# haan6/fm-for-online-recommendation

Measured on AMD Instinct MI355X. Metric: samples/sec online-FM (Criteo-39-field, k=16) FTRL-proximal, higher is better.
Workload: dtype f32

## Files before the change

fm-for-online-recommendation_amd/csrc/fmx_kernels.hip:

```cpp

#include <type_traits>

#include "fmx_common.h"

namespace fmxd {

thread_local char g_err[512] = "";

int fail(int code, const char *fmt, ...) {
  va_list ap;
  va_start(ap, fmt);
  vsnprintf(g_err, sizeof(g_err), fmt, ap);
  va_end(ap);
  return code;
}

int check_launch(const char *what) {
  hipError_t e = hipGetLastError();
  if (e != hipSuccess) return fail(FMX_ERR_LAUNCH, "%s: %s", what, hipGetErrorString(e));
  return FMX_OK;
}

}

namespace {

#include "fmx_sort.inc"

__device__ __forceinline__ void st_sc1(float *p, float v) { __hip_atomic_store(p, v, __ATOMIC_RELAXED, __HIP_MEMORY_SCOPE_AGENT); }
__device__ __forceinline__ float ld_sc1(const float *p) {
  return __hip_atomic_load(p, __ATOMIC_RELAXED, __HIP_MEMORY_SCOPE_AGENT);
}
__device__ __forceinline__ float4 ld_sc1_4(const float *p) { return {ld_sc1(p), ld_sc1(p + 1), ld_sc1(p + 2), ld_sc1(p + 3)}; }
typedef float v4f __attribute__((ext_vector_type(4)));
__device__ __forceinline__ void st_sc1_4(float *p, float4 v) {
  const v4f x = {v.x, v.y, v.z, v.w};
  asm volatile("global_store_dwordx4 %0, %1, off sc1\n\ts_nop 1" ::"v"(p), "v"(x) : "memory");
}
__device__ __forceinline__ void store_part_sc1(float *rec, int q, int kp, float4 cV, float4 cA, float cw) {
  st_sc1_4(rec + 4 * q, cV);
  st_sc1_4(rec + kp + 4 * q, cA);
  if (q == 0) st_sc1(rec + 2 * kp, cw);
}

struct FwdArgs {
  const float *rows;
  const int64_t *foff;
  const float *bias;
  const int32_t *idx;
  const float *xv;
  const float *y;
  fmx_fwd_out_t out;
  fmx_hyper_t h;
  int32_t B, F, kp, stride, zoff, loss_kind;
  int32_t ldS, ld1;
  float inv_b;
  const int32_t *fcols, *fbase;
  int32_t Fc;
};

template <int LPR, int LAYOUT>
__device__ __forceinline__ void forward_finish(const FwdArgs &a, const int b, const int lane, float4 s, float4 ss, float fo, bool bad,
                                               const float y_early, const float bias0_early, const float bias1_early) {
  const int q = lane % LPR;
  const int kp = LPR * 4;
  if (bad && a.out.error) *a.out.error = 1;

#define FMX_BFLY(M)                               \
  if (LPR <= M) {                                 \
    s = s + xor_lane_f4<M>(s, lane);              \
    ss = ss + xor_lane_f4<M>(ss, lane);           \
    fo += xor_lane_f<M>(fo, lane);                \
  }
  FMX_BFLY(1) FMX_BFLY(2) FMX_BFLY(4) FMX_BFLY(8) FMX_BFLY(16) FMX_BFLY(32)
#undef FMX_BFLY
  const float4 bi = 0.5f * (s * s - ss);
  float sbi = (bi.x + bi.y) + (bi.z + bi.w);
#pragma unroll
  for (int m = 1; m < LPR; m <<= 1) sbi += __shfl_xor(sbi, m);
  fo = __shfl(fo, 0);

  if (lane < LPR) {
    if (a.out.S) *reinterpret_cast<float4 *>(a.out.S + (size_t)b * a.ldS + 4 * q) = s;
    if (a.out.bi) *reinterpret_cast<float4 *>(a.out.bi + (size_t)b * kp + 4 * q) = bi;
  }
  if (lane == 0) {
    float bias;
    if (LAYOUT == FMX_LAYOUT_WEIGHTS) bias = bias0_early;
    else bias = ftrl_w(bias0_early, bias1_early, a.h);
    const float z = fo + sbi + bias;
    if (a.out.sfirst) a.out.sfirst[b] = fo;
    if (a.out.sbi) a.out.sbi[b] = sbi;
    if (a.out.logit) a.out.logit[b] = z;
    if (a.loss_kind != FMX_LOSS_NONE) {
      const float y = y_early;
      float loss, dz;
      if (a.loss_kind == FMX_LOSS_BCE_LOGITS) {
        loss = bcewl(z, y);
        dz = (sigmoidf_(z) - y) * a.inv_b;
      } else {
        const float p = sigmoidf_(z);
        loss = bcewl(p, y);
        dz = (sigmoidf_(p) - y) * p * (1.f - p) * a.inv_b;
      }
      if (a.out.loss) a.out.loss[(size_t)b * a.ld1] = loss;
      if (a.out.dz) a.out.dz[(size_t)b * a.ld1] = dz;
    }
  }
}

template <int LPR, int LAYOUT, int NPASS, bool MAPPED = false>
__device__ __forceinline__ void forward_sample(const FwdArgs &a, const int b, const int lane) {
  constexpr int SLOTS = WAVE / LPR;
  constexpr int NP = NPASS > 0 ? NPASS : 1;
  const int slot = lane / LPR, q = lane % LPR;
  const int kp = LPR * 4;

  float4 s = splat(0.f), ss = splat(0.f);
  float fo = 0.f;
  bool bad = false;
  const float y_early = a.loss_kind != FMX_LOSS_NONE ? a.y[b] : 0.f;
  const float bias0_early = a.bias[0];
  const float bias1_early = LAYOUT == FMX_LAYOUT_WEIGHTS ? 0.f : a.bias[1];
  __builtin_amdgcn_sched_barrier(0);
  const int n_outer = NPASS > 0 ? 1 : (a.F + SLOTS - 1) / SLOTS;
  for (int it = 0; it < n_outer; ++it) {
    uint32_t li[NP];
    float x[NP];
    int64_t lo[NP];
    uint32_t vocab[NP];
    bool live[NP];
    const float *xsrc = a.xv ? a.xv : reinterpret_cast<const float *>(a.idx);
    const bool has_x = a.xv != nullptr;
    float xl[NP];
    int64_t hi[NP];
    int fc[NP];
#pragma unroll
    for (int p = 0; p < NP; ++p) {
      const int f = (it * NP + p) * SLOTS + slot;
      live[p] = f < a.F;
      fc[p] = live[p] ? f : a.F - 1;
    }
#pragma unroll
    for (int p = 0; p < NP; ++p) {
      lo[p] = a.foff[fc[p]];
      hi[p] = a.foff[fc[p] + 1];
    }
#pragma unroll
    for (int p = 0; p < NP; ++p) {
      size_t o = (size_t)b * a.F + fc[p];
      uint32_t fb = 0u;
      if (MAPPED) {
        o = (size_t)b * a.Fc + (a.fcols ? a.fcols[fc[p]] : fc[p]);
        fb = a.fbase ? (uint32_t)a.fbase[fc[p]] : 0u;
      }
      li[p] = (uint32_t)a.idx[o] - fb;
      xl[p] = xsrc[o];
    }
#pragma unroll
    for (int p = 0; p < NP; ++p) {
      x[p] = has_x ? xl[p] : 1.f;
      vocab[p] = (uint32_t)(hi[p] - lo[p]);
    }
    float4 r0[NP];
    float rw[NP];
    bool ok[NP];
#pragma unroll
    for (int p = 0; p < NP; ++p) {
      ok[p] = live[p] && li[p] < vocab[p];
      const float *rp = a.rows + (size_t)(lo[p] + (ok[p] ? li[p] : 0u)) * a.stride;
      r0[p] = *reinterpret_cast<const float4 *>(rp + 4 * q);
      rw[p] = rp[kp];
    }
    __builtin_amdgcn_sched_barrier(0);
#pragma unroll
    for (int p = 0; p < NP; ++p) {
      const float4 e = x[p] * r0[p];
      const float f1 = ok[p] ? rw[p] * x[p] : 0.f;
      if (ok[p]) {
        s = s + e;
        ss = ss + e * e;
        fo += f1;
      }
      bad = bad || (!MAPPED && live[p] && !ok[p]);
      if (live[p] && a.out.first && q == 0) a.out.first[(size_t)b * a.F + (it * NP + p) * SLOTS + slot] = f1;
    }
  }
  forward_finish<LPR, LAYOUT>(a, b, lane, s, ss, fo, bad, y_early, bias0_early, bias1_early);
}

template <int LPR, int LAYOUT, int NPASS, bool MAPPED = false>
__global__ __launch_bounds__(256) void k_fm_forward(FwdArgs a) {
  __builtin_amdgcn_s_setprio(3);
  const int b = blockIdx.x * (blockDim.x >> 6) + (threadIdx.x >> 6);
  if (b >= a.B) return;
  forward_sample<LPR, LAYOUT, NPASS, MAPPED>(a, b, threadIdx.x & 63);
}

struct PartArgs {
  const float *rows;
  const int64_t *foff;
  const int32_t *fcols, *fbase;
  const int32_t *idx;
  const float *xv;
  float *rec;
  int32_t *error;
  int32_t B, F, Fc, stride, sl_log2, group;
};

template <int LPR, int NPASS>
__global__ __launch_bounds__(256) void k_fm_forward_part(PartArgs a) {
  constexpr int SLOTS = WAVE / LPR;
  constexpr int kp = LPR * 4, REC = 2 * kp + 4;
  const int lane = threadIdx.x & 63;
  const int slot = lane / LPR, q = lane % LPR;
  const int SL = 1 << a.sl_log2;
  const int slot_l = slot & (SL - 1);
  const int wave = blockIdx.x * (blockDim.x >> 6) + (threadIdx.x >> 6);
  const int b = wave * (SLOTS >> a.sl_log2) + (slot >> a.sl_log2);
  const bool valid = b < a.B;
  const int f0 = (int)blockIdx.y * NPASS * SL;
  const bool pieces = a.fcols || a.fbase;
  uint32_t li[NPASS], vocab[NPASS];
  float x[NPASS], xl[NPASS];
  int64_t lo[NPASS], hi[NPASS];
  bool live[NPASS], ok[NPASS];
  int fc[NPASS];
  const float *xsrc = a.xv ? a.xv : reinterpret_cast<const float *>(a.idx);
  const bool has_x = a.xv != nullptr;
  const int bc = valid ? b : 0;
#pragma unroll
  for (int p = 0; p < NPASS; ++p) {
    const int f = f0 + p * SL + slot_l;
    live[p] = valid && f < a.F;
    fc[p] = f < a.F ? f : a.F - 1;
  }
  int colp[NPASS];
  uint32_t fb[NPASS];
#pragma unroll
  for (int p = 0; p < NPASS; ++p) {
    lo[p] = a.foff[fc[p]];
    hi[p] = a.foff[fc[p] + 1];
    colp[p] = a.fcols ? a.fcols[fc[p]] : fc[p];
    fb[p] = a.fbase ? (uint32_t)a.fbase[fc[p]] : 0u;
  }
#pragma unroll
  for (int p = 0; p < NPASS; ++p) {
    const size_t o = (size_t)bc * a.Fc + colp[p];
    li[p] = (uint32_t)a.idx[o] - fb[p];
    xl[p] = xsrc[o];
  }
#pragma unroll
  for (int p = 0; p < NPASS; ++p) {
    x[p] = has_x ? xl[p] : 1.f;
    vocab[p] = (uint32_t)(hi[p] - lo[p]);
  }
  float4 r0[NPASS];
  float rw[NPASS];
#pragma unroll
  for (int p = 0; p < NPASS; ++p) {
    ok[p] = live[p] && li[p] < vocab[p];
    const float *rp = a.rows + (size_t)(lo[p] + (ok[p] ? li[p] : 0u)) * a.stride;
    r0[p] = *reinterpret_cast<const float4 *>(rp + 4 * q);
    rw[p] = rp[kp];
  }
  __builtin_amdgcn_sched_barrier(0);
  float4 s = splat(0.f), ss = splat(0.f);
  float fo = 0.f;
  bool bad = false;
#pragma unroll
  for (int p = 0; p < NPASS; ++p) {
    const float4 e = x[p] * r0[p];
    if (ok[p]) {
      s = s + e;
      ss = ss + e * e;
      fo += rw[p] * x[p];
    }
    bad = bad || (!pieces && live[p] && !ok[p]);
  }
  if (bad && a.error) *a.error = 1;
#define FMX_BFLY_L(M)                              \
  if (LPR <= M && (M / LPR) < SL) {                \
    s = s + xor_lane_f4<M>(s, lane);               \
    ss = ss + xor_lane_f4<M>(ss, lane);            \
    fo += xor_lane_f<M>(fo, lane);                 \
  }
  FMX_BFLY_L(1) FMX_BFLY_L(2) FMX_BFLY_L(4) FMX_BFLY_L(8) FMX_BFLY_L(16) FMX_BFLY_L(32)
#undef FMX_BFLY_L
  if (valid && slot_l == 0) {
    const int dst = b / a.group;
    float *r = a.rec + (((size_t)dst * gridDim.y + blockIdx.y) * a.group + (b - dst * a.group)) * REC;
    *reinterpret_cast<float4 *>(r + 4 * q) = s;
    *reinterpret_cast<float4 *>(r + kp + 4 * q) = ss;
    if (q == 0) *reinterpret_cast<float4 *>(r + 2 * kp) = float4{fo, 0.f, 0.f, 0.f};
  }
}

struct FinishArgs {
  const float *parts;
  int64_t rank_stride;
  const float *bias;
  const float *y;
  fmx_fwd_out_t out;
  fmx_hyper_t h;
  int32_t B, loss_kind, ldS, ld1;
  float inv_b;
};

template <int LPR, int LAYOUT, int G>
__global__ __launch_bounds__(256) void k_fm_forward_finish(FinishArgs a) {
  constexpr int SLOTS = WAVE / LPR;
  constexpr int kp = LPR * 4, REC = 2 * kp + 4;
  const int lane = threadIdx.x & 63;
  const int slot = lane / LPR, q = lane % LPR;
  const int b = (blockIdx.x * (blockDim.x >> 6) + (threadIdx.x >> 6)) * SLOTS + slot;
  const bool valid = b < a.B;
  const float y_early = (valid && a.loss_kind != FMX_LOSS_NONE) ? a.y[b] : 0.f;
  const float bias0 = a.bias[0];
  const float bias1 = LAYOUT == FMX_LAYOUT_WEIGHTS ? 0.f : a.bias[1];
  float4 s[G], ss[G];
  float fo[G];
#pragma unroll
  for (int r = 0; r < G; ++r) {
    s[r] = ss[r] = splat(0.f);
    fo[r] = 0.f;
    if (valid) {
      const float *p = a.parts + (size_t)r * a.rank_stride + (size_t)b * REC;
      s[r] = *reinterpret_cast<const float4 *>(p + 4 * q);
      ss[r] = *reinterpret_cast<const float4 *>(p + kp + 4 * q);
      if (q == 0) fo[r] = p[2 * kp];
    }
  }
#pragma unroll
  for (int st = 1; st < G; st <<= 1) {
#pragma unroll
    for (int r = 0; r < G; r += 2 * st) {
      s[r] = s[r] + s[r + st];
      ss[r] = ss[r] + ss[r + st];
      fo[r] += fo[r + st];
    }
  }
  const float4 bi = 0.5f * (s[0] * s[0] - ss[0]);
  float sbi = (bi.x + bi.y) + (bi.z + bi.w);
#pragma unroll
  for (int m = 1; m < LPR; m <<= 1) sbi += __shfl_xor(sbi, m);
  if (!valid) return;
  if (a.out.S) *reinterpret_cast<float4 *>(a.out.S + (size_t)b * a.ldS + 4 * q) = s[0];
  if (a.out.bi) *reinterpret_cast<float4 *>(a.out.bi + (size_t)b * kp + 4 * q) = bi;
  if (q == 0) {
    float bias;
    if (LAYOUT == FMX_LAYOUT_WEIGHTS) bias = bias0;
    else bias = ftrl_w(bias0, bias1, a.h);
    const float z = fo[0] + sbi + bias;
    if (a.out.sfirst) a.out.sfirst[b] = fo[0];
    if (a.out.sbi) a.out.sbi[b] = sbi;
    if (a.out.logit) a.out.logit[b] = z;
    if (a.loss_kind != FMX_LOSS_NONE) {
      const float y = y_early;
      float loss, dz;
      if (a.loss_kind == FMX_LOSS_BCE_LOGITS) {
        loss = bcewl(z, y);
        dz = (sigmoidf_(z) - y) * a.inv_b;
      } else {
        const float pp = sigmoidf_(z);
        loss = bcewl(pp, y);
        dz = (sigmoidf_(pp) - y) * pp * (1.f - pp) * a.inv_b;
      }
      if (a.out.loss) a.out.loss[(size_t)b * a.ld1] = loss;
      if (a.out.dz) a.out.dz[(size_t)b * a.ld1] = dz;
    }
  }
}

struct UpdArgs {
  float *rows;
  const int64_t *foff;
  float *bias;
  const uint32_t *sorted;
  float *parts;
  int32_t *meta;
  const float *xv;
  const float *S;
  const float *dz_first;
  const float *dz_bi;
  const float *gbi;
  const float *loss_b;
  float *loss_out;
  int32_t *step_counter;
  fmx_hyper_t h;
  int32_t B, F, Bp, bbits, kp, stride, zoff;
  int32_t ldS, ld1;
  int32_t ldG;
  const int32_t *cols;
  const int32_t *fcols;
  int32_t Fx;
  float *red;
  uint32_t seq;
  int32_t *error;
  float inv_b;
};

constexpr int LEAD_NONE = 0, LEAD_CLOSES = 1, LEAD_THROUGH = 2;

__device__ __forceinline__ void st16(float *p, float4 v) {
  typedef float f4v __attribute__((ext_vector_type(4)));
  __builtin_nontemporal_store(f4v{v.x, v.y, v.z, v.w}, reinterpret_cast<f4v *>(p));
}
__device__ __forceinline__ void st4(float *p, float v) { __builtin_nontemporal_store(v, p); }

constexpr int RED_SLICE = 4096;
__host__ __device__ inline int red_slices(int B) { return (B + RED_SLICE - 1) / RED_SLICE; }

template <int LAYOUT, int RULE>
__device__ __forceinline__ void apply_bias_and_loss(const UpdArgs &a, float db, float ls) {
  if (LAYOUT == FMX_LAYOUT_WEIGHTS) {
    st4(a.bias, apply_rule<RULE>(a.bias[0], db, a.h));
  } else if (LAYOUT == FMX_LAYOUT_MOMENTS) {
    float p = a.bias[0], m = a.bias[1], v = a.bias[2];
    moments_upd<RULE>(p, m, v, db, a.h);
    st4(a.bias, p);
    if (RULE == FMX_RULE_ADAM) st4(a.bias + 1, m);
    st4(a.bias + 2, v);
  } else {
    float z = a.bias[0], n = a.bias[1];
    const float w = ftrl_w(z, n, a.h);
    ftrl_upd(z, n, w, db, a.h);
    st4(a.bias, z);
    st4(a.bias + 1, n);
  }
  if (a.loss_b && a.loss_out) {
    int i = 0;
    if (a.step_counter) {
      i = *a.step_counter;
      *a.step_counter = i + 1;
    }
    a.loss_out[i] = ls * a.inv_b;
  }
}

template <int LAYOUT, int RULE>
__device__ void finish_bias_and_loss(const UpdArgs &a, int R, bool poll) {
  __shared__ float part[2 * 16];
  const int t = threadIdx.x;
  bool failed = false;
  if (t < R) {
    const v4f *src = reinterpret_cast<const v4f *>(a.red) + t;
    v4f g = {0.f, 0.f, 0.f, 0.f};
    if (poll) {
      for (int spin = 0;; ++spin) {
        asm volatile("global_load_dwordx4 %0, %1, off sc1\n\ts_waitcnt vmcnt(0)" : "=v"(g) : "v"(src) : "memory");
        if (__float_as_uint(g.z) == a.seq) break;
        if (spin >= (1 << 20)) {
          failed = true;
          break;
        }
        __builtin_amdgcn_s_sleep(1);
      }
    } else {
      g = *src;
    }
    part[2 * t] = g.x;
    part[2 * t + 1] = g.y;
  }
  if (failed && a.error) *a.error = 2;
  __syncthreads();
  if (t == 0) {
    float db = 0.f, ls = 0.f;
    for (int r = 0; r < R; ++r) {
      db += part[2 * r];
      ls += part[2 * r + 1];
    }
    apply_bias_and_loss<LAYOUT, RULE>(a, db, ls);
  }
}

template <int LAYOUT, int RULE, bool INL>
__device__ void bias_and_loss(const UpdArgs &a, int r) {
  __shared__ float sm[256];
  const int R = red_slices(a.B);
  const int first = r * RED_SLICE, n = (a.B - first) < RED_SLICE ? (a.B - first) : RED_SLICE;
  const float db = block_sum(a.dz_first + (size_t)first * a.ld1, n, a.ld1, sm);
  float ls = 0.f;
  if (a.loss_b && a.loss_out) ls = block_sum(a.loss_b + (size_t)first * a.ld1, n, a.ld1, sm);
  if (R == 1) {
    if (threadIdx.x == 0) apply_bias_and_loss<LAYOUT, RULE>(a, db, ls);
    return;
  }
  if (threadIdx.x == 0) st_sc1_4(a.red + 4 * r, float4{db, ls, __uint_as_float(a.seq), 0.f});
  if (INL && r == 0) finish_bias_and_loss<LAYOUT, RULE>(a, R, true);
}

struct RowRegs {
  float4 v;
  float4 z, n;
  float4 fo;
};

template <int LAYOUT, int RULE>
__device__ __forceinline__ RowRegs load_row(const float *rp, int q, int kp, int zoff) {
// ... 1940 lines not shown

  const int REP = 8, n_ev = 5;
  const int n_groups = (n_steps + REP - 1) / REP;
  const size_t F = (size_t)n_cols(table);
  const size_t region = align_up((size_t)B * table->kp + 2 * (size_t)B, 64);
  float *tmp = nullptr;
  hipEvent_t *ev = nullptr;
  int rc = FMX_OK;
  {
    const Detour detour(st == nullptr ? side_for_current_device() : nullptr, st);
    st = detour.st;
    if (n_groups > 0 && hipMalloc(&tmp, REP * region * sizeof(float)) != hipSuccess)
      return fail(FMX_ERR_LAUNCH, "hipMalloc (measuring mode)");
    ev = new hipEvent_t[(size_t)n_groups * n_ev];
    for (int i = 0; i < n_groups * n_ev; ++i) (void)hipEventCreate(&ev[i]);
    for (int g = 0; g < n_groups && rc == FMX_OK; ++g) {
      const int first = g * REP, n = (n_steps - first) < REP ? (n_steps - first) : REP;
      hipEvent_t *e = ev + (size_t)g * n_ev;
      (void)hipEventRecord(e[0], st);
      rc = sort_pool(table, idx_pool, n_pool, B, first, n, w, w.sorted, fwd->error, st);
      (void)hipEventRecord(e[1], st);
      for (int r = 0; r < n && rc == FMX_OK; ++r) {
        const int j = (first + r) % n_pool;
        fmx_fwd_out_t fr = *fwd;
        fr.S = tmp + (size_t)r * region;
        fr.dz = fr.S + (size_t)B * table->kp;
        fr.loss = fr.dz + B;
        fr.sample_ld = 0;
        rc = forward_impl(table, hyper, idx_pool + (size_t)j * B * F, nullptr, y_pool + (size_t)j * B, B, loss_kind, inv_b, &fr, st);
      }
      (void)hipEventRecord(e[2], st);
      for (int r = 0; r < n && rc == FMX_OK; ++r) {
        const float *S = tmp + (size_t)r * region, *dz = S + (size_t)B * table->kp;
        fmx_hyper_t hs = hyper_for(hyper, rule);
        hs.step += first + r;
        rc = update_impl(table, &hs, rule, w, w.sorted + (size_t)r * w.sorted_stride, nullptr, S, dz, dz, nullptr, B, dz + B, inv_b,
                         loss_out ? loss_out + first + r : nullptr, st, nullptr, 0, fwd->error);
      }
      (void)hipEventRecord(e[3], st);
      (void)hipEventRecord(e[4], st);
    }
    (void)hipStreamSynchronize(st);
  }
  for (int k = 0; k < 4; ++k) kernel_ms[k] = 0.f;
  if (rc == FMX_OK && n_groups > 0) {
    double t_sort = 0, t_fwd = 0, t_upd = 0, t_pair = 0;
    for (int g = 0; g < n_groups; ++g) {
      hipEvent_t *e = ev + (size_t)g * n_ev;
      float pair = 0.f, ms[3] = {0.f, 0.f, 0.f};
      (void)hipEventElapsedTime(&pair, e[3], e[4]);
      for (int k = 0; k < 3; ++k) (void)hipEventElapsedTime(&ms[k], e[k], e[k + 1]);
      t_pair += pair;
      t_sort += fmaxf(ms[0] - pair, 0.f);
      t_fwd += fmaxf(ms[1] - pair, 0.f);
      t_upd += fmaxf(ms[2] - pair, 0.f);
    }
    kernel_ms[0] = (float)(t_sort / n_groups * n_steps);
    kernel_ms[1] = (float)t_fwd;
    kernel_ms[2] = (float)t_upd;
    kernel_ms[3] = (float)(t_pair / n_groups * n_steps);
  }
  for (int i = 0; i < n_groups * n_ev; ++i) (void)hipEventDestroy(ev[i]);
  delete[] ev;
  if (tmp) (void)hipFree(tmp);
  return rc;
}

int fmx_fm_online_run(const fmx_table_t *table, const fmx_hyper_t *hyper, int32_t rule, int32_t loss_kind,
                      const int32_t *idx, const float *xv, const float *y, int32_t N, uint8_t *pred_out, float *loss_out,
                      int32_t *error, fmx_stream_t stream) {
  if (int rc = check_table(table)) return rc;
  if (int rc = check_rule(table, rule)) return rc;
  if (mapped(table)) return fail(FMX_ERR_UNSUPPORTED, "fmx_fm_online_run: tables whose fields are pieces of index columns are not taken");
  if (N < 0) return fail(FMX_ERR_ARG, "fmx_fm_online_run: N must be >= 0");
  if (N == 0) return FMX_OK;
  if (!hyper || !idx || !y || !pred_out) return fail(FMX_ERR_ARG, "fmx_fm_online_run: null argument");
  if (int rc = check_adam(hyper, rule, N)) return rc;
  if (loss_kind != FMX_LOSS_BCE_LOGITS && loss_kind != FMX_LOSS_BCE_SIGMOID) return fail(FMX_ERR_ARG, "fit needs a loss");
  const int lpr = lpr_of(table->kp), slots = WAVE / lpr;
  const int np = (table->n_fields + slots - 1) / slots;
  if (np > 4)
    return fail(FMX_ERR_UNSUPPORTED, "fmx_fm_online_run: %d fields at kp = %d exceed the %d rows one wavefront holds", table->n_fields,
                table->kp, 4 * slots);
  OnlineArgs a;
  a.rows = table->rows;
  a.foff = table->field_offsets;
  a.bias = table->bias;
  a.idx = idx;
  a.xv = xv;
  a.y = y;
  a.pred = pred_out;
  a.loss = loss_out;
  a.error = error;
  a.h = hyper_for(hyper, rule);
  a.h.alpha = 1.0f / hyper->alpha;
  a.N = N;
  a.F = table->n_fields;
  a.stride = table->row_stride;
  a.zoff = table->z_offset;
  a.loss_kind = loss_kind;
  hipStream_t st = static_cast<hipStream_t>(stream);
  with_lpr(table->kp, [&](auto LPR) {
    with_rule(rule, [&](auto LAYOUT, auto RULE) { launch_online_np<LPR, LAYOUT, RULE>(a, np, st); });
  });
  return check_launch("k_fm_online");
}

static int mlp_launch(const fmx_mlp_t *mlp, MlpArgs &a, int32_t B, int32_t kp, fmx_stream_t stream, const char *who) {
  if (!mlp || !mlp->params) return fail(FMX_ERR_ARG, "%s: null mlp", who);
  if (mlp->n_layers < 1 || mlp->n_layers > MLP_MAX_L || mlp->hidden < 1 || mlp->hidden > MLP_MAX_W || mlp->k < 1 ||
      mlp->k > MLP_MAX_W || B < 1 || B > MLP_MAX_B || kp < mlp->k)
    return fail(FMX_ERR_UNSUPPORTED, "%s: needs B <= %d, k <= %d, hidden <= %d, layers <= %d (got B=%d k=%d hidden=%d layers=%d)", who,
                MLP_MAX_B, MLP_MAX_W, MLP_MAX_W, MLP_MAX_L, B, mlp->k, mlp->hidden, mlp->n_layers);
  a.params = mlp->params;
  a.B = B;
  a.k = mlp->k;
  a.kp = kp;
  a.hidden = mlp->hidden;
  a.n_layers = mlp->n_layers;
  hipLaunchKernelGGL(k_mlp_small, dim3(1), dim3(256), 0, static_cast<hipStream_t>(stream), a);
  return check_launch("k_mlp_small");
}

int fmx_online_run_mlp(const fmx_table_t *table, const fmx_hyper_t *hyper, int32_t rule, int32_t loss_kind,
                       const fmx_mlp_t *mlp, int32_t hedge, int32_t fm_term, float hedge_b, float hedge_s, float *alpha,
                       const int32_t *idx, const float *xv, const float *y, int32_t N, void *workspace, int64_t workspace_bytes,
                       const fmx_fwd_out_t *fwd, float *scratch, float *pred_out, fmx_stream_t stream) {
  if (int rc = check_table(table)) return rc;
  if (!hyper || !mlp || !idx || !y || !workspace || !fwd || !scratch || !pred_out)
    return fail(FMX_ERR_ARG, "fmx_online_run_mlp: null argument");
  if (mapped(table)) return fail(FMX_ERR_UNSUPPORTED, "fmx_online_run_mlp: tables whose fields are pieces of index columns are not taken");
  if (!fwd->S || !fwd->bi || !fwd->sfirst || !fwd->logit) return fail(FMX_ERR_ARG, "fmx_online_run_mlp: fwd needs S, bi, sfirst, logit");
  if (!aligned16(workspace) || !aligned16(scratch)) return fail(FMX_ERR_ALIGN, "workspace and scratch must be 16-byte aligned");
  if (hedge && !alpha) return fail(FMX_ERR_ARG, "fmx_online_run_mlp: Hedge needs alpha");
  if (!hedge) {
    if (adaptive_rule(rule)) return refuse_adaptive(rule, "fmx_online_run_mlp (fit mode)");
    if (int rc = check_rule(table, rule)) return rc;
    if (rule != FMX_RULE_SIGNADAM && rule != FMX_RULE_SGD) return fail(FMX_ERR_ARG, "fmx_online_run_mlp: rule must be SIGNADAM or SGD");
    if (loss_kind != FMX_LOSS_BCE_LOGITS && loss_kind != FMX_LOSS_BCE_SIGMOID) return fail(FMX_ERR_ARG, "fit needs a loss");
    if (mlp->k > MLP_MAX_W - 1) return fail(FMX_ERR_UNSUPPORTED, "fmx_online_run_mlp: k <= %d", MLP_MAX_W - 1);
    if (int rc = check_sort_geometry(table, 1)) return rc;
  } else if (mlp->k + mlp->n_layers > MLP_MAX_W) {
    return fail(FMX_ERR_UNSUPPORTED, "fmx_online_run_mlp: k + layers <= %d", MLP_MAX_W);
  }
  if (N < 0) return fail(FMX_ERR_ARG, "N must be >= 0");
  hipStream_t st = static_cast<hipStream_t>(stream);
  {
    long long n_params = 0;
    for (int l = 0; l < mlp->n_layers; ++l) n_params += (long long)mlp->hidden * (l == 0 ? mlp->k : mlp->hidden) + mlp->hidden;
    const int lpr = lpr_of(table->kp), slots = WAVE / lpr;
    const bool tables_ok = hedge || table->layout == FMX_LAYOUT_WEIGHTS;
    if (tune().online_persistent && n_params <= ONLINE_MLP_MAX_PARAMS && table->n_fields <= 4 * slots && tables_ok &&
        mlp->hidden <= MLP_MAX_W && mlp->n_layers <= MLP_MAX_L && mlp->k <= MLP_MAX_W - 1 && N > 0) {
      OnlineMlpArgs a;
      a.rows = table->rows;
      a.foff = table->field_offsets;
      a.bias = table->bias;
      a.idx = idx;
      a.xv = xv;
      a.y = y;
      a.pred = pred_out;
      a.error = fwd->error;
      a.params = mlp->params;
      a.alpha = alpha;
      a.h = hyper_for(hyper, -1);
      a.h.alpha = 1.0f / hyper->alpha;
      a.hedge_b = hedge_b;
      a.hedge_s = hedge_s;
      a.N = N;
      a.F = table->n_fields;
      a.stride = table->row_stride;
      a.zoff = table->z_offset;
      a.n_params = (int32_t)n_params;
      a.k = mlp->k;
      a.hidden = mlp->hidden;
      a.n_layers = mlp->n_layers;
      a.hedge = hedge;
      a.fm_term = fm_term;
      a.rule = rule;
      a.loss_kind = loss_kind;
      const int kernel_rule = table->layout == FMX_LAYOUT_FTRL ? FMX_RULE_FTRL : rule == FMX_RULE_SGD ? FMX_RULE_SGD : FMX_RULE_SIGNADAM;
      with_lpr(table->kp, [&](auto LPR) {
        with_rule_wf(kernel_rule, [&](auto LAYOUT, auto RULE) { launch_online_mlp_k<LPR, LAYOUT, RULE>(a, st); });
      });
      return check_launch("k_online_mlp");
    }
  }
  if (int rc = check_workspace(table, 1, workspace, workspace_bytes, "fmx_online_run_mlp")) return rc;
  const Workspace w = carve(table, 1, workspace);
  const size_t F = (size_t)table->n_fields;
  fmx_fwd_out_t f1 = *fwd;
  f1.sample_ld = 0;
  float *dz = scratch, *gbi = scratch + 8;
  for (int i = 0; i < N; ++i) {
    const int32_t *idx_i = idx + (size_t)i * F;
    const float *xv_i = xv ? xv + (size_t)i * F : nullptr;
    if (int rc = forward_impl(table, hyper, idx_i, xv_i, nullptr, 1, FMX_LOSS_NONE, 1.0f, &f1, st)) return rc;
    MlpArgs a{};
    a.bi = fwd->bi;
    a.base = fm_term ? fwd->logit : fwd->sfirst;
    if (!fm_term) {
      a.base_bias = table->bias;
      a.base_bias_ftrl = table->layout == FMX_LAYOUT_FTRL;
      a.h_table = hyper_for(hyper, -1);
      a.h_table.alpha = 1.0f / hyper->alpha;
    }
    a.y = y + i;
    a.pred_out = pred_out + i;
    a.h = hyper_for(hyper, -1);
    a.inv_b = 1.0f;
    if (hedge) {
      a.alpha = alpha;
      a.hedge_b = hedge_b;
      a.hedge_s = hedge_s;
      a.mode = MLP_MODE_HEDGE;
    } else {
      a.dz_out = dz;
      a.gbi_out = gbi;
      a.mode = MLP_MODE_FIT;
      a.rule = rule;
      a.loss_kind = loss_kind;
    }
    if (int rc = mlp_launch(mlp, a, 1, table->kp, stream, "fmx_online_run_mlp")) return rc;
    if (hedge) continue;
    if (int rc = sort_impl(table, idx_i, 1, w.sorted, w.runs, fwd->error, st)) return rc;
    if (int rc = update_impl(table, hyper, rule, w, w.sorted, xv_i, fwd->S, dz, fm_term ? dz : nullptr, gbi, 1, nullptr, 1.0f, nullptr,
                             st, nullptr, 0, fwd->error))
      return rc;
  }
  return FMX_OK;
}

int fmx_mlp_forward(const fmx_mlp_t *mlp, const float *bi, int32_t kp, const float *base, int32_t B, float *out,
                    float *layers_out, fmx_stream_t stream) {
  if (!bi || !base || (!out && !layers_out)) return fail(FMX_ERR_ARG, "fmx_mlp_forward: null argument");
  MlpArgs a{};
  a.bi = bi;
  a.base = base;
  a.out = out;
  a.layers_out = layers_out;
  a.mode = MLP_MODE_FORWARD;
  return mlp_launch(mlp, a, B, kp, stream, "fmx_mlp_forward");
}

int fmx_mlp_fit(const fmx_mlp_t *mlp, const fmx_hyper_t *hyper, int32_t rule, int32_t loss_kind, const float *bi, int32_t kp,
                const float *base, const float *y, int32_t B, float inv_b, float *dz_out, float *gbi_out, float *loss_out,
                fmx_stream_t stream) {
  if (adaptive_rule(rule)) return refuse_adaptive(rule, "fmx_mlp_fit");
  if (!hyper || !bi || !base || !y || !dz_out || !gbi_out) return fail(FMX_ERR_ARG, "fmx_mlp_fit: null argument");
  if (rule != FMX_RULE_SIGNADAM && rule != FMX_RULE_SGD) return fail(FMX_ERR_ARG, "fmx_mlp_fit: rule must be SIGNADAM or SGD");
  if (loss_kind != FMX_LOSS_BCE_LOGITS && loss_kind != FMX_LOSS_BCE_SIGMOID) return fail(FMX_ERR_ARG, "fmx_mlp_fit needs a loss");
  if (mlp && mlp->k > MLP_MAX_W - 1) return fail(FMX_ERR_UNSUPPORTED, "fmx_mlp_fit: k <= %d", MLP_MAX_W - 1);
  MlpArgs a{};
  a.bi = bi;
  a.base = base;
  a.y = y;
  a.dz_out = dz_out;
  a.gbi_out = gbi_out;
  a.out = loss_out;
  a.h = hyper_for(hyper, -1);
  a.mode = MLP_MODE_FIT;
  a.rule = rule;
  a.loss_kind = loss_kind;
  a.inv_b = inv_b;
  return mlp_launch(mlp, a, B, kp, stream, "fmx_mlp_fit");
}

int fmx_mlp_hedge_fit(const fmx_mlp_t *mlp, float lr, float hedge_b, float hedge_s, float *alpha, const float *bi, int32_t kp,
                      const float *base, const float *y, int32_t B, float *losses_out, fmx_stream_t stream) {
  if (!alpha || !bi || !base || !y) return fail(FMX_ERR_ARG, "fmx_mlp_hedge_fit: null argument");
  if (mlp && mlp->k + mlp->n_layers > MLP_MAX_W) return fail(FMX_ERR_UNSUPPORTED, "fmx_mlp_hedge_fit: k + layers <= %d", MLP_MAX_W);
  MlpArgs a{};
  a.bi = bi;
  a.base = base;
  a.y = y;
  a.alpha = alpha;
  a.layers_out = losses_out;
  a.h.lr = lr;
  a.hedge_b = hedge_b;
  a.hedge_s = hedge_s;
  a.mode = MLP_MODE_HEDGE;
  a.inv_b = 1.0f / (float)B;
  return mlp_launch(mlp, a, B, kp, stream, "fmx_mlp_hedge_fit");
}

int fmx_gather_read(const void *buf, int64_t bytes, int32_t row_bytes, int64_t n_rows_read, uint32_t seed, float *sink, fmx_stream_t stream) {
  if (!buf || !sink || bytes < 128 || n_rows_read < 1) return fail(FMX_ERR_ARG, "fmx_gather_read: bad buffer / count");
  if (row_bytes != 64 && row_bytes != 128) return fail(FMX_ERR_ARG, "fmx_gather_read: rows of 64 or 128 bytes");
  if (!aligned16(buf)) return fail(FMX_ERR_ALIGN, "fmx_gather_read: buffer must be 16-byte aligned");
  const int lpr = row_bytes / 16;
  const uint64_t n_rows = (uint64_t)bytes / (uint64_t)row_bytes;
  const int64_t threads = n_rows_read * lpr;
  const dim3 grid((unsigned)((threads + 255) / 256)), block(256);
  hipStream_t st = static_cast<hipStream_t>(stream);
  if (lpr == 4) hipLaunchKernelGGL((k_gather_read<4>), grid, block, 0, st, static_cast<const float4 *>(buf), n_rows, n_rows_read, seed, sink);
  else hipLaunchKernelGGL((k_gather_read<8>), grid, block, 0, st, static_cast<const float4 *>(buf), n_rows, n_rows_read, seed, sink);
  return check_launch("k_gather_read");
}

#ifdef FMX_STAMPS
int fmx_debug_update_stamps(unsigned long long *host_out) {
  return hipMemcpyFromSymbol(host_out, HIP_SYMBOL(g_upd_stamps), sizeof(unsigned long long) * 8192 * 6) == hipSuccess ? FMX_OK : FMX_ERR_LAUNCH;
}
#endif

int fmx_stream_read(const void *buf, int64_t bytes, float *sink, fmx_stream_t stream) {
  if (!buf || !sink || bytes < 16 || bytes % 16) return fail(FMX_ERR_ARG, "fmx_stream_read: bad buffer");
  if (!aligned16(buf)) return fail(FMX_ERR_ALIGN, "fmx_stream_read: buffer must be 16-byte aligned");
  hipLaunchKernelGGL(k_stream_read, dim3(256 * 8), dim3(256), 0, static_cast<hipStream_t>(stream),
                     static_cast<const float4 *>(buf), bytes / 16, sink);
  return check_launch("k_stream_read");
}

}
```

Measured before the change: 185.3 million.

## Load per-field metadata once per wave lane and broadcast row offsets via shuffles

The forward kernel now has each lane load the offsets, index and value for one field, computes the validated row index, then broadcasts it to the lanes that handle that field with 64-bit shuffles, instead of every lane redundantly loading the metadata. The xv presence check becomes a compile-time template parameter, and the FTRL bias computation is moved so it overlaps the row gathers. Optional timestamp instrumentation is also added behind a compile flag. This cuts redundant scalar loads and address math on the critical path at the cost of extra cross-lane shuffles.

```diff
diff --git a/fm-for-online-recommendation_amd/csrc/fmx_kernels.hip b/fm-for-online-recommendation_amd/csrc/fmx_kernels.hip
--- a/fm-for-online-recommendation_amd/csrc/fmx_kernels.hip
+++ b/fm-for-online-recommendation_amd/csrc/fmx_kernels.hip
@@ -59,9 +59,21 @@
   int32_t Fc;
 };
 
-template <int LPR, int LAYOUT>
+#ifdef FMX_STAMPS
+__device__ unsigned long long g_fwd_stamps[8192 * 6];
+#define FMX_FSTAMP(slot_, dep_)                                                                                     \
+  do {                                                                                                              \
+    unsigned long long t_;                                                                                          \
+    asm volatile("s_memrealtime %0\n\ts_waitcnt lgkmcnt(0)" : "=s"(t_) : "v"(dep_) : "memory");                      \
+    if (lane == 0 && b < 8192) g_fwd_stamps[(size_t)b * 6 + (slot_)] = t_;                                           \
+  } while (0)
+#else
+#define FMX_FSTAMP(slot_, dep_) do {} while (0)
+#endif
+
+template <int LPR>
 __device__ __forceinline__ void forward_finish(const FwdArgs &a, const int b, const int lane, float4 s, float4 ss, float fo, bool bad,
-                                               const float y_early, const float bias0_early, const float bias1_early) {
+                                               const float y_early, const float bias) {
   const int q = lane % LPR;
   const int kp = LPR * 4;
   if (bad && a.out.error) *a.out.error = 1;
@@ -79,15 +91,13 @@
 #pragma unroll
   for (int m = 1; m < LPR; m <<= 1) sbi += __shfl_xor(sbi, m);
   fo = __shfl(fo, 0);
+  FMX_FSTAMP(3, sbi);
 
   if (lane < LPR) {
     if (a.out.S) *reinterpret_cast<float4 *>(a.out.S + (size_t)b * a.ldS + 4 * q) = s;
     if (a.out.bi) *reinterpret_cast<float4 *>(a.out.bi + (size_t)b * kp + 4 * q) = bi;
   }
   if (lane == 0) {
-    float bias;
-    if (LAYOUT == FMX_LAYOUT_WEIGHTS) bias = bias0_early;
-    else bias = ftrl_w(bias0_early, bias1_early, a.h);
     const float z = fo + sbi + bias;
     if (a.out.sfirst) a.out.sfirst[b] = fo;
     if (a.out.sbi) a.out.sbi[b] = sbi;
@@ -103,18 +113,28 @@
         loss = bcewl(p, y);
         dz = (sigmoidf_(p) - y) * p * (1.f - p) * a.inv_b;
       }
+      FMX_FSTAMP(4, dz);
       if (a.out.loss) a.out.loss[(size_t)b * a.ld1] = loss;
       if (a.out.dz) a.out.dz[(size_t)b * a.ld1] = dz;
     }
-  }
-}
-
-template <int LPR, int LAYOUT, int NPASS, bool MAPPED = false>
+    FMX_FSTAMP(5, z);
+  }
+}
+
+__device__ __forceinline__ int64_t shfl64(int64_t v, int src) {
+  const int lo = __shfl((int)(uint32_t)v, src), hi = __shfl((int)(v >> 32), src);
+  return (int64_t)(((uint64_t)(uint32_t)hi << 32) | (uint32_t)lo);
+}
+constexpr int64_t ROW_ABSENT = int64_t(1) << 62;
+
+template <int LPR, int LAYOUT, int NPASS, bool MAPPED, bool HAS_X>
 __device__ __forceinline__ void forward_sample(const FwdArgs &a, const int b, const int lane) {
   constexpr int SLOTS = WAVE / LPR;
   constexpr int NP = NPASS > 0 ? NPASS : 1;
+  constexpr int NW = NPASS > 0 ? (NP * SLOTS + WAVE - 1) / WAVE : 1;
   const int slot = lane / LPR, q = lane % LPR;
   const int kp = LPR * 4;
+  FMX_FSTAMP(0, lane);
 
   float4 s = splat(0.f), ss = splat(0.f);
   float fo = 0.f;
@@ -123,54 +143,65 @@
   const float bias0_early = a.bias[0];
   const float bias1_early = LAYOUT == FMX_LAYOUT_WEIGHTS ? 0.f : a.bias[1];
   __builtin_amdgcn_sched_barrier(0);
+  float bias = 0.f;
   const int n_outer = NPASS > 0 ? 1 : (a.F + SLOTS - 1) / SLOTS;
   for (int it = 0; it < n_outer; ++it) {
-    uint32_t li[NP];
-    float x[NP];
-    int64_t lo[NP];
-    uint32_t vocab[NP];
-    bool live[NP];
-    const float *xsrc = a.xv ? a.xv : reinterpret_cast<const float *>(a.idx);
-    const bool has_x = a.xv != nullptr;
-    float xl[NP];
-    int64_t hi[NP];
-    int fc[NP];
-#pragma unroll
-    for (int p = 0; p < NP; ++p) {
-      const int f = (it * NP + p) * SLOTS + slot;
-      live[p] = f < a.F;
-      fc[p] = live[p] ? f : a.F - 1;
-    }
-#pragma unroll
-    for (int p = 0; p < NP; ++p) {
-      lo[p] = a.foff[fc[p]];
-      hi[p] = a.foff[fc[p] + 1];
-    }
-#pragma unroll
-    for (int p = 0; p < NP; ++p) {
-      size_t o = (size_t)b * a.F + fc[p];
+    int fl[NW];
+    bool wlive[NW];
+    int64_t lo[NW], hi[NW];
+    uint32_t li[NW];
+    float xl[NW];
+#pragma unroll
+    for (int w = 0; w < NW; ++w) {
+      const int f = (NPASS > 0 ? w * WAVE : it * SLOTS) + lane;
+      wlive[w] = f < a.F;
+      fl[w] = wlive[w] ? f : a.F - 1;
+    }
+#pragma unroll
+    for (int w = 0; w < NW; ++w) {
+      lo[w] = a.foff[fl[w]];
+      hi[w] = a.foff[fl[w] + 1];
+    }
+#pragma unroll
+    for (int w = 0; w < NW; ++w) {
+      size_t o = (size_t)b * a.F + fl[w];
       uint32_t fb = 0u;
       if (MAPPED) {
-        o = (size_t)b * a.Fc + (a.fcols ? a.fcols[fc[p]] : fc[p]);
-        fb = a.fbase ? (uint32_t)a.fbase[fc[p]] : 0u;
+        o = (size_t)b * a.Fc + (a.fcols ? a.fcols[fl[w]] : fl[w]);
+        fb = a.fbase ? (uint32_t)a.fbase[fl[w]] : 0u;
       }
-      li[p] = (uint32_t)a.idx[o] - fb;
-      xl[p] = xsrc[o];
-    }
-#pragma unroll
-    for (int p = 0; p < NP; ++p) {
-      x[p] = has_x ? xl[p] : 1.f;
-      vocab[p] = (uint32_t)(hi[p] - lo[p]);
-    }
+      li[w] = (uint32_t)a.idx[o] - fb;
+      xl[w] = HAS_X ? a.xv[o] : 1.f;
+    }
+    int64_t row[NW];
+#pragma unroll
+    for (int w = 0; w < NW; ++w) {
+      const bool okw = wlive[w] && li[w] < (uint32_t)(hi[w] - lo[w]);
+      row[w] = lo[w] + (okw ? li[w] : 0u);
+      if (!okw) row[w] |= ROW_ABSENT;
+      bad = bad || (!MAPPED && wlive[w] && !okw);
+    }
+    FMX_FSTAMP(1, (uint32_t)row[0]);
+    float x[NP];
     float4 r0[NP];
     float rw[NP];
-    bool ok[NP];
+    bool ok[NP], live[NP];
 #pragma unroll
     for (int p = 0; p < NP; ++p) {
-      ok[p] = live[p] && li[p] < vocab[p];
-      const float *rp = a.rows + (size_t)(lo[p] + (ok[p] ? li[p] : 0u)) * a.stride;
+      const int f = NPASS > 0 ? p * SLOTS + slot : slot;
+      const int w = NPASS > 0 ? (p * SLOTS) / WAVE : 0;
+      live[p] = (NPASS > 0 ? f : it * SLOTS + f) < a.F;
+      const int64_t r = shfl64(row[w], f % WAVE);
+      x[p] = HAS_X ? __shfl(xl[w], f % WAVE) : 1.f;
+      ok[p] = live[p] && !(r & ROW_ABSENT);
+      const float *rp = a.rows + (size_t)(r & ~ROW_ABSENT) * a.stride;
       r0[p] = *reinterpret_cast<const float4 *>(rp + 4 * q);
       rw[p] = rp[kp];
+    }
+    __builtin_amdgcn_sched_barrier(0);
+    if (it == 0) {
+      bias = LAYOUT == FMX_LAYOUT_WEIGHTS ? bias0_early : ftrl_w(bias0_early, bias1_early, a.h);
+      asm volatile("" ::"v"(bias));
     }
     __builtin_amdgcn_sched_barrier(0);
 #pragma unroll
@@ -182,11 +213,11 @@
         ss = ss + e * e;
         fo += f1;
       }
-      bad = bad || (!MAPPED && live[p] && !ok[p]);
       if (live[p] && a.out.first && q == 0) a.out.first[(size_t)b * a.F + (it * NP + p) * SLOTS + slot] = f1;
     }
-  }
-  forward_finish<LPR, LAYOUT>(a, b, lane, s, ss, fo, bad, y_early, bias0_early, bias1_early);
+    FMX_FSTAMP(2, s.x + ss.x + fo);
+  }
+  forward_finish<LPR>(a, b, lane, s, ss, fo, bad, y_early, bias);
 }
 
 template <int LPR, int LAYOUT, int NPASS, bool MAPPED = false>
@@ -194,7 +225,8 @@
   __builtin_amdgcn_s_setprio(3);
   const int b = blockIdx.x * (blockDim.x >> 6) + (threadIdx.x >> 6);
   if (b >= a.B) return;
-  forward_sample<LPR, LAYOUT, NPASS, MAPPED>(a, b, threadIdx.x & 63);
+  if (a.xv) forward_sample<LPR, LAYOUT, NPASS, MAPPED, true>(a, b, threadIdx.x & 63);
+  else forward_sample<LPR, LAYOUT, NPASS, MAPPED, false>(a, b, threadIdx.x & 63);
 }
 
 struct PartArgs {
@@ -2741,6 +2773,9 @@
 int fmx_debug_update_stamps(unsigned long long *host_out) {
   return hipMemcpyFromSymbol(host_out, HIP_SYMBOL(g_upd_stamps), sizeof(unsigned long long) * 8192 * 6) == hipSuccess ? FMX_OK : FMX_ERR_LAUNCH;
 }
+int fmx_debug_forward_stamps(unsigned long long *host_out) {
+  return hipMemcpyFromSymbol(host_out, HIP_SYMBOL(g_fwd_stamps), sizeof(unsigned long long) * 8192 * 6) == hipSuccess ? FMX_OK : FMX_ERR_LAUNCH;
+}
 #endif
 
 int fmx_stream_read(const void *buf, int64_t bytes, float *sink, fmx_stream_t stream) {
```

New measurement: 190.1 million, median of 6. +2.6%, better.
